# sephiroce/srf

Measured on AMD Instinct MI355X. Metric: acoustic frames/sec through SRF (123-d fbank, 3-iter DR) at 1/2/4/8 MI355X, higher is better.
Workload: dtype fp32; 1 GPU; wsj_c4: SRF L=6 PH=CH=16 DIM=32 LPAD=RPAD=2 DR iter=3, train step (fwd+bwd+allreduce+Adam); utterances_per_gpu=28, frames_per_utterance=800, global_batch=28, parallelism=dp1, launch=hipgraph (fwd+CTC+bwd)

## Files before the change

srf_amd/csrc/cnnfe.hip:

```cpp
#include <algorithm>
#include <type_traits>
#include <cmath>
#include <cstdlib>

#include "srf_common.h"
#include "srf_reduce.h"
#include "srf_rng.h"
#include "../../include/srf.h"

namespace {

constexpr int C = 64;
constexpr float kBnEps = 1e-3f;
constexpr float kBnMomentum = 0.99f;

struct Dims {
  int B, T, Fin;
  int T1, F1, T2, F2;
  int pt1, pf1, pt2, pf2;
};

inline int same_out(int n) { return (n + 1) / 2; }
inline int same_pad_before(int n) {
  const int out = same_out(n);
// ... 167 lines not shown
                                                           const float* __restrict__ gamma,
                                                           const float* __restrict__ beta,
                                                           float* __restrict__ mmean, float* __restrict__ mvar,
                                                           int training, float* __restrict__ stats,
                                                           const float* __restrict__ ymax, int nymax) {
  __shared__ float sh[3][16][C];
  __shared__ float ysh[16], ab[2][C];
  const int c = threadIdx.x & (C - 1), r = threadIdx.x >> 6;
  if (ymax != nullptr) {
    float m = 0.f;
    for (int k = threadIdx.x; k < nymax; k += 1024) m = fmaxf(m, ymax[k]);
#pragma unroll
    for (int o = 32; o >= 1; o >>= 1) m = fmaxf(m, __shfl_xor(m, o, 64));
    if (c == 0) ysh[r] = m;
  }
  float n = 0.f, mu = 0.f, m2 = 0.f;
  if (training)
#pragma unroll 8
    for (int k = r; k < nparts; k += 16)
      chan_merge(n, mu, m2, part[((size_t)k * 3 + 0) * C + c], part[((size_t)k * 3 + 1) * C + c],
                 part[((size_t)k * 3 + 2) * C + c]);
  sh[0][r][c] = n; sh[1][r][c] = mu; sh[2][r][c] = m2;
  __syncthreads();
  if (r == 0) {
    float mean, var;
    if (training) {
      for (int q = 1; q < 16; ++q) chan_merge(n, mu, m2, sh[0][q][c], sh[1][q][c], sh[2][q][c]);
      mean = mu;
      var = m2 / n;
      mmean[c] = mmean[c] * kBnMomentum + mean * (1.f - kBnMomentum);
      mvar[c] = mvar[c] * kBnMomentum + (n > 1.f ? var * n / (n - 1.f) : var) * (1.f - kBnMomentum);
    } else {
      mean = mmean[c];
      var = mvar[c];
    }
    const float rstd = 1.f / sqrtf(var + kBnEps);
    const float scale = gamma[c] * rstd;
    const float shift = beta[c] - mean * scale;
    stats[0 * C + c] = mean;
    stats[1 * C + c] = rstd;
    stats[2 * C + c] = scale;
    stats[3 * C + c] = shift;
    ab[0][c] = fabsf(scale);
    ab[1][c] = fabsf(shift);
  }
  if (ymax == nullptr) return;
  __syncthreads();
  if (threadIdx.x == 0) {
    float y = ysh[0], sa = 0.f, sb = 0.f;
    for (int q = 1; q < 16; ++q) y = fmaxf(y, ysh[q]);
    for (int q = 0; q < C; ++q) {
      sa = fmaxf(sa, ab[0][q]);
      sb = fmaxf(sb, ab[1][q]);
    }
    const int e = srf_split_exp(sa * y + sb);
    stats[4 * C + 0] = srf_exp2i(e);
    stats[4 * C + 1] = srf_exp2i(-e);
  }
}

typedef __bf16 cbf8 __attribute__((ext_vector_type(8)));
typedef float cf16 __attribute__((ext_vector_type(16)));

__device__ __forceinline__ cf16 mfma32bf(const cbf8& a, const cbf8& b, const cf16& c) {
  return __builtin_amdgcn_mfma_f32_32x32x16_bf16(a, b, c, 0, 0, 0);
}
typedef _Float16 ch8 __attribute__((ext_vector_type(8)));
__device__ __forceinline__ cf16 mfma32h(const ch8& a, const ch8& b, const cf16& c) {
  return __builtin_amdgcn_mfma_f32_32x32x16_f16(a, b, c, 0, 0, 0);
}

__device__ __forceinline__ void split8v(const float (&v)[8], cbf8& p1, cbf8& p2, cbf8& p3) {
#pragma unroll
  for (int k = 0; k < 8; ++k) {
    const __bf16 a1 = (__bf16)v[k];
    const float r = v[k] - (float)a1;
    const __bf16 a2 = (__bf16)r;
    p1[k] = a1;
    p2[k] = a2;
    p3[k] = (__bf16)(r - (float)a2);
  }
}

__device__ __forceinline__ void pack_w2_f16_body(int idx, const float* __restrict__ ka, const float* __restrict__ kb,
                                                 _Float16* __restrict__ wp2, float* __restrict__ wsc) {
  const int n = idx >> 6, cin = idx & 63;
  const float* k = n < C ? ka : kb;
  const int co = n % C;
  float v[9], m = 0.f;
#pragma unroll
  for (int tap = 0; tap < 9; ++tap) {
    v[tap] = k[((size_t)tap * C + cin) * C + co];
    m = fmaxf(m, fabsf(v[tap]));
  }
#pragma unroll
  for (int o = 32; o >= 1; o >>= 1) m = fmaxf(m, __shfl_xor(m, o, 64));
  const int e = srf_split_exp(m);
  const float sc = srf_exp2i(e);
  const size_t plane = (size_t)9 * 2 * C * C;
#pragma unroll
  for (int tap = 0; tap < 9; ++tap) {
    _Float16 h1, h2;
    srf_split2h(v[tap] * sc, h1, h2);
    const size_t o = ((size_t)tap * 2 * C + n) * C + cin;
    wp2[o] = h1;
    wp2[plane + o] = h2;
  }
  if (cin == 0) wsc[n] = srf_exp2i(-e);
}

constexpr int kC2BStride = 24;
constexpr int kC2Waves = 4;
constexpr int kC2Px = 32 * kC2Waves;
constexpr int kC2BLoads = 2 * 2 * C * 2 / (64 * kC2Waves);

__global__ __launch_bounds__(64 * kC2Waves) __attribute__((amdgpu_waves_per_eu(2))) void conv2_fwd32_kernel(
    const float* __restrict__ y1, const float* __restrict__ stats1, const int* __restrict__ inp_len, Dims d,
    const _Float16* __restrict__ wp2, const float* __restrict__ wsc, const float* __restrict__ ba,
    const float* __restrict__ bb, int training, float drop_p, unsigned long long seed,
    const unsigned long long* __restrict__ seed_src, float* __restrict__ y2, unsigned char* __restrict__ sel2,
    float* __restrict__ part) {
  seed = srf_step_seed(seed, seed_src);
  __shared__ __attribute__((aligned(16))) _Float16 Bs[2][2][2 * C * kC2BStride];
  __shared__ __attribute__((aligned(16))) float ss[2][C];
  __shared__ float red[3][kC2Waves][2 * 32];
  const int tid = threadIdx.x;
  const int lane = tid & 63, wv = tid >> 6;
  const int r = lane & 31, h = lane >> 5;
  const int P2 = d.B * d.T2 * d.F2;
  const int p0 = blockIdx.x * kC2Px;
  const size_t plane = (size_t)9 * 2 * C * C;
  if (tid < 2 * C) ss[tid >> 6][tid & 63] = stats1[(2 + (tid >> 6)) * C + (tid & 63)] * stats1[4 * C];

  const int pa = p0 + 32 * wv + r;
  const bool alive = pa < P2;
  const int pc = min(pa, P2 - 1);
  const int af2 = pc % d.F2, at2 = (pc / d.F2) % d.T2, ab = pc / (d.F2 * d.T2);
  const int alen1 = ceil_div_len(inp_len[ab], 2);

  auto load_b = [&](int kk, ch8 (&bv)[kC2BLoads]) {
    const int tap = kk >> 2, kb = kk & 3;
#pragma unroll
    for (int q = 0; q < kC2BLoads; ++q) {
      const int idx = q * 64 * kC2Waves + tid;
      const int pl = idx >> 8, rem = idx & 255, n = rem >> 1, half = rem & 1;
      bv[q] = *reinterpret_cast<const ch8*>(wp2 + pl * plane + ((size_t)tap * 2 * C + n) * C + 16 * kb + 8 * half);
    }
  };
  auto store_b = [&](int buf, const ch8 (&bv)[kC2BLoads]) {
#pragma unroll
    for (int q = 0; q < kC2BLoads; ++q) {
      const int idx = q * 64 * kC2Waves + tid;
      const int pl = idx >> 8, rem = idx & 255, n = rem >> 1, half = rem & 1;
      *reinterpret_cast<ch8*>(&Bs[buf][pl][n * kC2BStride + 8 * half]) = bv[q];
    }
  };
  auto load_a = [&](int kk, f4 (&av)[2], bool& ok) {
    const int tap = kk >> 2, kb = kk & 3;
    const int dt = tap / 3, df = tap - dt * 3;
    const int t1 = 2 * at2 - d.pt2 + dt, f1 = 2 * af2 - d.pf2 + df;
    ok = alive && t1 >= 0 && t1 < d.T1 && f1 >= 0 && f1 < d.F1 && t1 < alen1;
    const int t1c = min(max(t1, 0), d.T1 - 1), f1c = min(max(f1, 0), d.F1 - 1);
    const float* src = y1 + (((size_t)ab * d.T1 + t1c) * d.F1 + f1c) * C + 16 * kb + 8 * h;
    av[0] = *reinterpret_cast<const f4*>(src);
    av[1] = *reinterpret_cast<const f4*>(src + 4);
  };

  cf16 acc[4];
#pragma unroll
  for (int nt = 0; nt < 4; ++nt) acc[nt] = cf16{};
  auto compute = [&](int kk, int buf, const f4 (&av)[2], bool aok) {
    ch8 a1, a2;
    {
      const int c0 = 16 * (kk & 3) + 8 * h;
#pragma unroll
      for (int q = 0; q < 8; ++q) {
        const float x = q < 4 ? av[0][q] : av[1][q - 4];
        _Float16 h1, h2;
        srf_split2h(aok ? x * ss[0][c0 + q] + ss[1][c0 + q] : 0.f, h1, h2);
        a1[q] = h1;
        a2[q] = h2;
      }
    }
#pragma unroll
    for (int nt = 0; nt < 4; ++nt) {
      const int nrow = (nt >> 1) * C + 32 * (nt & 1) + r;
      const ch8 b1 = *reinterpret_cast<const ch8*>(&Bs[buf][0][nrow * kC2BStride + 8 * h]);
      const ch8 b2 = *reinterpret_cast<const ch8*>(&Bs[buf][1][nrow * kC2BStride + 8 * h]);
      cf16 c = acc[nt];
      c = mfma32h(a2, b1, c);
      c = mfma32h(a1, b2, c);
      c = mfma32h(a1, b1, c);
      acc[nt] = c;
    }
  };
  ch8 bvA[kC2BLoads], bvB[kC2BLoads];
  f4 avA[2], avB[2], avC[2];
  bool okA, okB, okC;
  load_b(0, bvA);
  load_a(0, avA, okA);
  load_b(1, bvB);
  load_a(1, avB, okB);
  store_b(0, bvA);
  __syncthreads();
  for (int kk = 0; kk < 36; kk += 2) {
    {
      const f4 a0[2] = {avA[0], avA[1]};
      const bool ok0 = okA;
      if (kk + 2 < 36) {
        load_b(kk + 2, bvA);
        load_a(kk + 2, avA, okA);
      }
      compute(kk, 0, a0, ok0);
      store_b(1, bvB);
      __syncthreads();
    }
    {
      const f4 a1v[2] = {avB[0], avB[1]};
      const bool ok1 = okB;
      if (kk + 3 < 36) {
        load_b(kk + 3, bvB);
        load_a(kk + 3, avB, okB);
      }
      compute(kk + 1, 1, a1v, ok1);
      if (kk + 2 < 36) store_b(0, bvA);
      __syncthreads();
    }
  }
  (void)avC;
  (void)okC;

  const float keep_scale = 1.f / (1.f - drop_p);
  const float inv_b = stats1[4 * C + 1];
#pragma unroll
  for (int g = 0; g < 2; ++g) {
    const int c = 32 * g + r;
    const float bia = ba[c], bib = bb[c];
    const float sca = wsc[c] * inv_b, scb = wsc[C + c] * inv_b;
    float n = 0.f, mean = 0.f, m2 = 0.f;
#pragma unroll
    for (int q = 0; q < 4; ++q)
#pragma unroll
      for (int v = 0; v < 4; ++v) {
        const int p = p0 + 32 * wv + 8 * q + 4 * h + v;
        if (p >= P2) continue;
        const int t2 = (p / d.F2) % d.T2, b = p / (d.F2 * d.T2);
        const size_t o = (size_t)p * C + c;
        float a = acc[g][4 * q + v] * sca + bia, bvv = acc[2 + g][4 * q + v] * scb + bib;
        if (training && drop_p > 0.f) {
          bool ka, kb;
          srf_keep2(seed, kStreamConv1a, o, drop_p, ka, kb);
          a *= ka ? keep_scale : 0.f;
          bvv *= kb ? keep_scale : 0.f;
        }
        const bool sel = a >= bvv;
        float y = sel ? a : bvv;
        if (t2 >= ceil_div_len(inp_len[b], 4)) y = 0.f;
        y2[o] = y;
        sel2[o] = sel ? 1 : 0;
        n += 1.f;
        const float delta = y - mean;
        mean += delta / n;
        m2 += delta * (y - mean);
      }
    {
      float nb, mb, qb, x;
      xpair32(n, x, nb);
      nb = h ? x : nb;
      xpair32(mean, x, mb);
      mb = h ? x : mb;
      xpair32(m2, x, qb);
      qb = h ? x : qb;
      if (h == 0) chan_merge(n, mean, m2, nb, mb, qb);
    }
    if (h == 0) {
      red[0][wv][g * 32 + r] = n;
      red[1][wv][g * 32 + r] = mean;
      red[2][wv][g * 32 + r] = m2;
    }
  }
  __syncthreads();
  if (tid < 2 * 32) {
    const int gc = tid;
    float n = red[0][0][gc], mean = red[1][0][gc], m2 = red[2][0][gc];
#pragma unroll
    for (int w = 1; w < kC2Waves; ++w) chan_merge(n, mean, m2, red[0][w][gc], red[1][w][gc], red[2][w][gc]);
    part[((size_t)blockIdx.x * 3 + 0) * C + gc] = n;
    part[((size_t)blockIdx.x * 3 + 1) * C + gc] = mean;
    part[((size_t)blockIdx.x * 3 + 2) * C + gc] = m2;
  }
}

__global__ void bn_apply_kernel(const float* __restrict__ y, const float* __restrict__ stats,
                                const int* __restrict__ inp_len, int B, int Tk, int Fk, int div,
                                float* __restrict__ out) {
  const int n4 = B * Tk * Fk * C / 4;
  for (int q = blockIdx.x * blockDim.x + threadIdx.x; q < n4; q += gridDim.x * blockDim.x) {
    const int c4 = (q * 4) % C;
    const int p = q * 4 / C;
    const int t = (p / Fk) % Tk;
    const int b = p / (Fk * Tk);
    f4 v = {0.f, 0.f, 0.f, 0.f};
    if (t < ceil_div_len(inp_len[b], div)) {
      const f4 x = reinterpret_cast<const f4*>(y)[q];
      v = x * *reinterpret_cast<const f4*>(stats + 2 * C + c4) + *reinterpret_cast<const f4*>(stats + 3 * C + c4);
    }
    reinterpret_cast<f4*>(out)[q] = v;
  }
}


constexpr int kBnPx = 16;
__device__ __forceinline__ f4 wave_sum_px(f4 v) {
#pragma unroll
  for (int o = 16; o <= 32; o <<= 1) {
    v.x += __shfl_xor(v.x, o, 64); v.y += __shfl_xor(v.y, o, 64);
    v.z += __shfl_xor(v.z, o, 64); v.w += __shfl_xor(v.w, o, 64);
  }
  return v;
}

__global__ __launch_bounds__(256) void bn_bwd_reduce_kernel(const float* __restrict__ g, const float* __restrict__ y,
                                                            const float* __restrict__ stats,
                                                            const int* __restrict__ inp_len, int B, int Tk, int Fk,
                                                            int div, float* __restrict__ part) {
  __shared__ f4 sh[2][4][C / 4];
  const int lane = threadIdx.x & 63, q = lane & 15, pg = lane >> 4;
  const int wave = __builtin_amdgcn_readfirstlane(threadIdx.x >> 6);
  const f4 mean = reinterpret_cast<const f4*>(stats)[q], rstd = reinterpret_cast<const f4*>(stats + C)[q];
  const int P = B * Tk * Fk;
  f4 s0 = {0.f, 0.f, 0.f, 0.f}, s1 = s0;
  for (int p0 = (blockIdx.x * 4 + wave) * kBnPx; p0 < P; p0 += gridDim.x * 4 * kBnPx) {
    constexpr int U = kBnPx / 4;
    f4 dy[U], yv[U];
    float m[U];
#pragma unroll
    for (int u = 0; u < U; ++u) {
      const int pu = p0 + 4 * u + pg;
      const int p = min(pu, P - 1);
      const int t = (p / Fk) % Tk;
// ... 35 lines not shown
    __bf16* __restrict__ wq3, _Float16* __restrict__ wq2h, float* __restrict__ wdsc, float* __restrict__ gmax) {
  if ((int)blockIdx.x >= nprep) {
    const int idx = (blockIdx.x - nprep) * blockDim.x + threadIdx.x;
    if (wq2h != nullptr) {
      if (idx < kPackW2tF16Threads) pack_w2t_f16_body(idx, pk_a, pk_b, wq2h, wdsc);
    } else if (idx < kPackW2tThreads) {
      pack_w2t_split_body(idx, pk_a, pk_b, wq3);
    }
    return;
  }
  seed = srf_step_seed(seed, seed_src);
  __shared__ f4 sh[2][4][C / 4];
  __shared__ float smax[4];
  const int lane = threadIdx.x & 63, q = lane & 15, pg = lane >> 4;
  const int wave = __builtin_amdgcn_readfirstlane(threadIdx.x >> 6);
  const int P = d.B * d.T2 * d.F2;
  const f4 mean = reinterpret_cast<const f4*>(stats2)[q], rstd = reinterpret_cast<const f4*>(stats2 + C)[q];
  const f4 gam = {gamma2[4 * q], gamma2[4 * q + 1], gamma2[4 * q + 2], gamma2[4 * q + 3]};
  const f4 sdy_n = reinterpret_cast<const f4*>(bnsum2)[q] / (float)P;
  const f4 sdyxh_n = reinterpret_cast<const f4*>(bnsum2 + C)[q] / (float)P;
  const float keep_scale = 1.f / (1.f - drop_p);
  f4 ga_s = {0.f, 0.f, 0.f, 0.f}, gb_s = ga_s;
  float gm = 0.f;
  for (int p0 = (blockIdx.x * 4 + wave) * kBnPx; p0 < P; p0 += nprep * 4 * kBnPx) {
    constexpr int U = kBnPx / 4;
    f4 gv[U], yv[U];
    unsigned sv[U];
    float m[U];
#pragma unroll
    for (int u = 0; u < U; ++u) {
      const int pu = p0 + 4 * u + pg;
      const int p = min(pu, P - 1);
      const int t = (p / d.F2) % d.T2;
      const int b = p / (d.F2 * d.T2);
      m[u] = (pu < P && t < ceil_div_len(inp_len[b], 4)) ? 1.f : 0.f;
      gv[u] = reinterpret_cast<const f4*>(g_out)[(size_t)p * (C / 4) + q];
      yv[u] = reinterpret_cast<const f4*>(y2)[(size_t)p * (C / 4) + q];
      sv[u] = reinterpret_cast<const unsigned*>(sel2)[(size_t)p * (C / 4) + q];
    }
#pragma unroll
    for (int u = 0; u < U; ++u) {
      const int pu = p0 + 4 * u + pg;
      if (pu >= P) continue;
      const size_t o0 = (size_t)pu * C + 4 * q;
      f4 ga, gb;
#pragma unroll
      for (int e = 0; e < 4; ++e) {
        const float gy = bn_bwd_elem(gv[u][e], yv[u][e], m[u], mean[e], rstd[e], gam[e], sdy_n[e], sdyxh_n[e]);
        const bool sel = ((sv[u] >> (8 * e)) & 0xffu) != 0;
        float a = sel ? gy : 0.f, bb = sel ? 0.f : gy;
        if (drop_p > 0.f) {
          bool ka, kb;
          srf_keep2(seed, kStreamConv1a, o0 + e, drop_p, ka, kb);
          a *= ka ? keep_scale : 0.f;
          bb *= kb ? keep_scale : 0.f;
        }
        ga[e] = a;
        gb[e] = bb;
        gm = fmaxf(gm, fmaxf(fabsf(a), fabsf(bb)));
      }
      reinterpret_cast<f4*>(g_ab + (size_t)pu * 2 * C)[q] = ga;
      reinterpret_cast<f4*>(g_ab + (size_t)pu * 2 * C + C)[q] = gb;
      ga_s += ga;
      gb_s += gb;
    }
  }
  ga_s = wave_sum_px(ga_s);
  gb_s = wave_sum_px(gb_s);
  if (pg == 0) { sh[0][wave][q] = ga_s; sh[1][wave][q] = gb_s; }
#pragma unroll
  for (int o = 32; o >= 1; o >>= 1) gm = fmaxf(gm, __shfl_xor(gm, o, 64));
  if (lane == 0) smax[wave] = gm;
  __syncthreads();
  if (threadIdx.x < 2 * (C / 4)) {
    const int k = threadIdx.x / (C / 4), qq = threadIdx.x % (C / 4);
    const f4 v = sh[k][0][qq] + sh[k][1][qq] + sh[k][2][qq] + sh[k][3][qq];
    reinterpret_cast<f4*>(part + (size_t)blockIdx.x * 2 * C + k * C)[qq] = v;
  }
  if (threadIdx.x == 0 && gmax != nullptr) gmax[blockIdx.x] = fmaxf(fmaxf(smax[0], smax[1]), fmaxf(smax[2], smax[3]));
}

struct DgCls {
  int boff[5];
};

__device__ __forceinline__ void pack_w2t_split_body(int idx, const float* __restrict__ ka,
                                                    const float* __restrict__ kb, __bf16* __restrict__ wq3) {
  const int n8 = idx % (2 * C / 8), cin = (idx / (2 * C / 8)) % C, tap = idx / (C * (2 * C / 8));
  const int n = 8 * n8;
  const float* k = (n < C ? ka : kb) + ((size_t)tap * C + cin) * C + (n % C);
  float v[8];
#pragma unroll
  for (int q = 0; q < 8; ++q) v[q] = k[q];
  cbf8 p1, p2, p3;
  split8v(v, p1, p2, p3);
  const size_t plane = (size_t)9 * C * 2 * C;
  const size_t o = ((size_t)tap * C + cin) * 2 * C + n;
  *reinterpret_cast<cbf8*>(wq3 + o) = p1;
  *reinterpret_cast<cbf8*>(wq3 + plane + o) = p2;
  *reinterpret_cast<cbf8*>(wq3 + 2 * plane + o) = p3;
}

__device__ __forceinline__ void pack_w2t_f16_body(int idx, const float* __restrict__ ka, const float* __restrict__ kb,
                                                  _Float16* __restrict__ wq2h, float* __restrict__ wdsc) {
  const int cin = idx >> 6, l = idx & 63;
  float v[9][2], m = 0.f;
#pragma unroll
  for (int tap = 0; tap < 9; ++tap)
#pragma unroll
    for (int u = 0; u < 2; ++u) {
      const int n = 2 * l + u;
      v[tap][u] = (n < C ? ka : kb)[((size_t)tap * C + cin) * C + (n % C)];
      m = fmaxf(m, fabsf(v[tap][u]));
    }
#pragma unroll
  for (int o = 32; o >= 1; o >>= 1) m = fmaxf(m, __shfl_xor(m, o, 64));
  const int e = srf_split_exp(m);
  const float sc = srf_exp2i(e);
  const size_t plane = (size_t)9 * C * 2 * C;
#pragma unroll
  for (int tap = 0; tap < 9; ++tap) {
    _Float16 h1[2], h2[2];
#pragma unroll
    for (int u = 0; u < 2; ++u) srf_split2h(v[tap][u] * sc, h1[u], h2[u]);
    const size_t o = ((size_t)tap * C + cin) * 2 * C + 2 * l;
    wq2h[o] = h1[0];
    wq2h[o + 1] = h1[1];
    wq2h[plane + o] = h2[0];
    wq2h[plane + o + 1] = h2[1];
  }
  if (l == 0) wdsc[cin] = srf_exp2i(-e);
}

constexpr int kD2Waves = 4;
constexpr int kD2Px = 32 * kD2Waves;

__device__ __forceinline__ int gab_exp(const float* __restrict__ gmax, int n) {
  __shared__ float wmx[16];
  const int tid = threadIdx.x, nw = (blockDim.x + 63) >> 6;
  float m = 0.f;
  for (int k = tid; k < n; k += blockDim.x) m = fmaxf(m, gmax[k]);
#pragma unroll
  for (int o = 32; o >= 1; o >>= 1) m = fmaxf(m, __shfl_xor(m, o, 64));
  if ((tid & 63) == 0) wmx[tid >> 6] = m;
  __syncthreads();
  for (int k = 0; k < nw; ++k) m = fmaxf(m, wmx[k]);
  return srf_split_exp(m);
}

template <bool H>
__global__ __launch_bounds__(64 * kD2Waves) __attribute__((amdgpu_waves_per_eu(2))) void conv2_dgrad32_kernel(
    const float* __restrict__ g_ab, const void* __restrict__ wqv, Dims d, DgCls cls, float* __restrict__ g_x1,
    const float* __restrict__ gmax, int ngmax, const float* __restrict__ wdsc) {
  using BT = std::conditional_t<H, _Float16, __bf16>;
  using V8 = std::conditional_t<H, ch8, cbf8>;
  constexpr int NPL = H ? 2 : 3;
  constexpr int BCH = NPL * C * 2;
  const BT* __restrict__ wq3 = static_cast<const BT*>(wqv);
  __shared__ __attribute__((aligned(16))) BT Bs[2][NPL][C * kC2BStride];
  const int tid = threadIdx.x;
  const int lane = tid & 63, wv = tid >> 6;
  const int r = lane & 31, h = lane >> 5;
  const int bid = blockIdx.x;
  const int c = (bid >= cls.boff[1]) + (bid >= cls.boff[2]) + (bid >= cls.boff[3]);
  const int qt = c >> 1, qf = c & 1;
  const int nkt = (d.T1 - qt + 1) / 2, nkf = (d.F1 - qf + 1) / 2;
  const int Pc = d.B * nkt * nkf;
  const int q0 = (bid - cls.boff[c]) * kD2Px;
  const int dt0 = (qt + d.pt2) & 1, df0 = (qf + d.pf2) & 1;
  const int ntf = (3 - df0 + 1) / 2, ntt = (3 - dt0 + 1) / 2;
  const int nkb = ntt * ntf * 8;
  const size_t plane = (size_t)9 * C * 2 * C;
  float sa = 1.f, inv_sa = 1.f;
  if constexpr (H) {
    const int ea = gab_exp(gmax, ngmax);
    sa = srf_exp2i(ea);
    inv_sa = srf_exp2i(-ea);
  }

  const int pa = q0 + 32 * wv + r;
  const bool alive = pa < Pc;
  const int pcl = min(pa, Pc - 1);
  const int akf = pcl % nkf, akt = (pcl / nkf) % nkt, ab = pcl / (nkf * nkt);
  const int at1 = qt + 2 * akt, af1 = qf + 2 * akf;
  auto tap_of = [&](int k) { return (dt0 + 2 * (k / ntf)) * 3 + df0 + 2 * (k % ntf); };

  constexpr int NBL = (BCH + 64 * kD2Waves - 1) / (64 * kD2Waves);
  auto load_b = [&](int kk, V8 (&bv)[NBL]) {
    const int tap = tap_of(kk >> 3), kb = kk & 7;
#pragma unroll
    for (int q = 0; q < NBL; ++q) {
      const int idx = min(q * 64 * kD2Waves + tid, BCH - 1);
      const int pl = idx / (2 * C), rem = idx % (2 * C), cin = rem >> 1, half = rem & 1;
      bv[q] = *reinterpret_cast<const V8*>(wq3 + pl * plane + ((size_t)tap * C + cin) * 2 * C + 16 * kb + 8 * half);
    }
  };
  auto store_b = [&](int buf, const V8 (&bv)[NBL]) {
#pragma unroll
    for (int q = 0; q < NBL; ++q) {
      const int idx = q * 64 * kD2Waves + tid;
      if (idx < BCH) {
        const int pl = idx / (2 * C), rem = idx % (2 * C), cin = rem >> 1, half = rem & 1;
        *reinterpret_cast<V8*>(&Bs[buf][pl][cin * kC2BStride + 8 * half]) = bv[q];
      }
    }
  };
  auto load_a = [&](int kk, f4 (&av)[2], bool& ok) {
    const int tap = tap_of(kk >> 3), kb = kk & 7;
    const int dt = tap / 3, df = tap - dt * 3;
    const int t2 = (at1 + d.pt2 - dt) >> 1, f2 = (af1 + d.pf2 - df) >> 1;
    ok = alive && t2 >= 0 && t2 < d.T2 && f2 >= 0 && f2 < d.F2;
    const int t2c = min(max(t2, 0), d.T2 - 1), f2c = min(max(f2, 0), d.F2 - 1);
    const float* src = g_ab + (((size_t)ab * d.T2 + t2c) * d.F2 + f2c) * 2 * C + 16 * kb + 8 * h;
    av[0] = *reinterpret_cast<const f4*>(src);
    av[1] = *reinterpret_cast<const f4*>(src + 4);
  };

  cf16 acc[2];
  acc[0] = cf16{};
  acc[1] = cf16{};
  auto compute = [&](int buf, const f4 (&av)[2], bool aok) {
    if constexpr (H) {
      ch8 a1, a2;
#pragma unroll
      for (int q = 0; q < 8; ++q) {
        const float v = aok ? (q < 4 ? av[0][q] : av[1][q - 4]) : 0.f;
        _Float16 h1, h2;
        srf_split2h(v * sa, h1, h2);
        a1[q] = h1;
        a2[q] = h2;
      }
#pragma unroll
      for (int nt = 0; nt < 2; ++nt) {
        const int nrow = 32 * nt + r;
        const ch8 b1 = *reinterpret_cast<const ch8*>(&Bs[buf][0][nrow * kC2BStride + 8 * h]);
        const ch8 b2 = *reinterpret_cast<const ch8*>(&Bs[buf][1][nrow * kC2BStride + 8 * h]);
        cf16 cc = acc[nt];
        cc = mfma32h(a2, b1, cc);
        cc = mfma32h(a1, b2, cc);
        cc = mfma32h(a1, b1, cc);
        acc[nt] = cc;
      }
      return;
    } else {
    cbf8 a1, a2, a3;
    {
      float v[8];
#pragma unroll
      for (int q = 0; q < 8; ++q) v[q] = aok ? (q < 4 ? av[0][q] : av[1][q - 4]) : 0.f;
      split8v(v, a1, a2, a3);
    }
#pragma unroll
    for (int nt = 0; nt < 2; ++nt) {
      const int nrow = 32 * nt + r;
      const cbf8 b1 = *reinterpret_cast<const cbf8*>(&Bs[buf][0][nrow * kC2BStride + 8 * h]);
      const cbf8 b2 = *reinterpret_cast<const cbf8*>(&Bs[buf][1][nrow * kC2BStride + 8 * h]);
      const cbf8 b3 = *reinterpret_cast<const cbf8*>(&Bs[buf][2][nrow * kC2BStride + 8 * h]);
      cf16 cc = acc[nt];
      cc = mfma32bf(a3, b1, cc);
      cc = mfma32bf(a1, b3, cc);
      cc = mfma32bf(a2, b2, cc);
      cc = mfma32bf(a2, b1, cc);
      cc = mfma32bf(a1, b2, cc);
      cc = mfma32bf(a1, b1, cc);
      acc[nt] = cc;
    }
    }
  };
  V8 bvA[NBL], bvB[NBL];
  f4 avA[2], avB[2];
  bool okA, okB;
  load_b(0, bvA);
  load_a(0, avA, okA);
  load_b(1, bvB);
  load_a(1, avB, okB);
  store_b(0, bvA);
  __syncthreads();
  for (int kk = 0; kk < nkb; kk += 2) {
    {
      const f4 a0[2] = {avA[0], avA[1]};
      const bool ok0 = okA;
      if (kk + 2 < nkb) {
        load_b(kk + 2, bvA);
        load_a(kk + 2, avA, okA);
      }
      compute(0, a0, ok0);
      store_b(1, bvB);
      __syncthreads();
    }
    {
      const f4 a1v[2] = {avB[0], avB[1]};
      const bool ok1 = okB;
      if (kk + 3 < nkb) {
        load_b(kk + 3, bvB);
        load_a(kk + 3, avB, okB);
      }
      compute(1, a1v, ok1);
      if (kk + 2 < nkb) store_b(0, bvA);
      __syncthreads();
    }
  }
  float osc[2] = {1.f, 1.f};
  if constexpr (H) {
    osc[0] = inv_sa * wdsc[r];
    osc[1] = inv_sa * wdsc[32 + r];
  }
#pragma unroll
  for (int q = 0; q < 4; ++q)
#pragma unroll
    for (int v = 0; v < 4; ++v) {
      const int p = q0 + 32 * wv + 8 * q + 4 * h + v;
      if (p >= Pc) continue;
      const int kf = p % nkf, kt = (p / nkf) % nkt, b = p / (nkf * nkt);
      float* dst = g_x1 + (((size_t)b * d.T1 + qt + 2 * kt) * d.F1 + qf + 2 * kf) * C + r;
      dst[0] = H ? acc[0][4 * q + v] * osc[0] : acc[0][4 * q + v];
      dst[32] = H ? acc[1][4 * q + v] * osc[1] : acc[1][4 * q + v];
    }
}

constexpr int kWgChunk = 32;

struct WgDiv {
  FastDiv f2, t2;
};

constexpr int kTpPx = 64;
template <bool H>
__global__ __launch_bounds__(256) void gab_split_t_kernel(const float* __restrict__ g_ab, int P2, int P2p,
                                                          void* __restrict__ gsTv, const float* __restrict__ gmax,
                                                          int ngmax) {
  __shared__ float tile[kTpPx][2 * C + 1];
  const int tid = threadIdx.x;
  const int p0 = blockIdx.x * kTpPx;
  float sa = 1.f;
  if constexpr (H) sa = srf_exp2i(gab_exp(gmax, ngmax));
  for (int k = tid; k < kTpPx * (2 * C / 4); k += 256) {
    const int px = k / (2 * C / 4), q = k % (2 * C / 4);
    const int p = p0 + px;
    const f4 v = p < P2 ? *reinterpret_cast<const f4*>(g_ab + (size_t)p * 2 * C + 4 * q) : f4{0.f, 0.f, 0.f, 0.f};
    tile[px][4 * q] = v.x;
    tile[px][4 * q + 1] = v.y;
    tile[px][4 * q + 2] = v.z;
    tile[px][4 * q + 3] = v.w;
  }
  __syncthreads();
  const size_t plane = (size_t)2 * C * P2p;
  for (int task = tid; task < 2 * C * (kTpPx / 8); task += 256) {
    const int o = task & 7, n = task >> 3;
    float v[8];
#pragma unroll
    for (int k = 0; k < 8; ++k) v[k] = tile[8 * o + k][n];
    if constexpr (H) {
      ch8 p1, p2;
#pragma unroll
      for (int k = 0; k < 8; ++k) {
        _Float16 h1, h2;
        srf_split2h(v[k] * sa, h1, h2);
        p1[k] = h1;
        p2[k] = h2;
      }
      _Float16* dst = static_cast<_Float16*>(gsTv) + (size_t)n * P2p + p0 + 8 * o;
      *reinterpret_cast<ch8*>(dst) = p1;
      *reinterpret_cast<ch8*>(dst + plane) = p2;
    } else {
      cbf8 p1, p2, p3;
      split8v(v, p1, p2, p3);
      __bf16* dst = static_cast<__bf16*>(gsTv) + (size_t)n * P2p + p0 + 8 * o;
      *reinterpret_cast<cbf8*>(dst) = p1;
      *reinterpret_cast<cbf8*>(dst + plane) = p2;
      *reinterpret_cast<cbf8*>(dst + 2 * plane) = p3;
    }
  }
}

constexpr int kW2Chunk = 32;
constexpr int kW2AStride = 96;

typedef short ws4 __attribute__((ext_vector_type(4)));

template <typename BT>
__device__ __forceinline__ ws4 lds_tr16(const BT* p) {
  return __builtin_amdgcn_ds_read_tr16_b64_v4i16(
      (__attribute__((address_space(3))) ws4*)(reinterpret_cast<uintptr_t>(p)));
}

template <bool H>
__global__ __launch_bounds__(256) __attribute__((amdgpu_waves_per_eu(2))) void conv2_wgrad32_kernel(
    const float* __restrict__ y1, const float* __restrict__ stats1, const int* __restrict__ inp_len,
    const void* __restrict__ gsTv, int P2p, Dims d, WgDiv dv, int nsplit, int split_len, float* __restrict__ part,
    const float* __restrict__ gmax, int ngmax) {
  using BT = std::conditional_t<H, _Float16, __bf16>;
  using V8 = std::conditional_t<H, ch8, cbf8>;
  constexpr int NPL = H ? 2 : 3;
  const BT* __restrict__ gsT3 = static_cast<const BT*>(gsTv);
  __shared__ __attribute__((aligned(16))) BT As[2][NPL][kW2Chunk * kW2AStride];
  float out_sc = 1.f;
// ... 460 lines not shown
  };
  const size_t op1 = take((size_t)conv1_blocks(d) * 3 * C * 4), op2 = take(nb2 * 3 * C * 4),
               owp = take((size_t)9 * 2 * C * C * 4), omg = take((size_t)kBnMerge * 3 * C * 4),
               owp2 = take((size_t)2 * 9 * 2 * C * C * 2), owsc = take((size_t)2 * C * 4),
               oym = take((size_t)conv1_blocks(d) * 4);
  char* b = static_cast<char*>(base);
  FwdWs w;
  w.wp2 = (_Float16*)(b + owp2);
  w.wsc = (float*)(b + owsc);
  w.ymax = (float*)(b + oym);
  w.merged = (float*)(b + omg);
  w.part1 = (float*)(b + op1);
  w.part2 = (float*)(b + op2);
  w.wp = (float*)(b + owp);
  w.bytes = off;
  return w;
}

int check_dims(int B, int T, int Fin, int nfilt) {
  SRF_REQUIRE(B > 0 && T > 0 && Fin > 0, "bad CNN-FE shape B=%d T=%d F=%d", B, T, Fin);
  SRF_REQUIRE(nfilt == C, "model-conv-filter-num must be %d (got %d)", C, nfilt);
  return SRF_OK;
}

}

extern "C" {

int srf_cnnfe_out_dims(int T, int feat_dim, int* T2, int* F2) {
  SRF_REQUIRE(T > 0 && feat_dim > 0 && T2 && F2, "bad arguments");
  Dims d = make_dims(1, T, feat_dim);
  *T2 = d.T2;
  *F2 = d.F2;
  return SRF_OK;
}

size_t srf_cnnfe_saved_bytes(int B, int T, int feat_dim, int nfilt) {
  (void)nfilt;
  return saved_layout(make_dims(B, T, feat_dim), nullptr).bytes;
}

size_t srf_cnnfe_fwd_workspace(int B, int T, int feat_dim, int nfilt) {
  (void)nfilt;
  return fwd_ws_layout(make_dims(B, T, feat_dim), nullptr).bytes;
}

int srf_cnnfe_fwd(const float* feats, const int* inp_len, int B, int T, int feat_dim, int nfilt,
                  const float* k0a, const float* b0a, const float* k0b, const float* b0b, const float* gamma0,
                  const float* beta0, const float* k1a, const float* b1a, const float* k1b, const float* b1b,
                  const float* gamma1, const float* beta1, float* mmean0, float* mvar0, float* mmean1, float* mvar1,
                  int training, float drop_p, unsigned long long seed, float* out, void* saved, size_t saved_bytes,
                  void* workspace, size_t workspace_bytes, void* stream) {
  int rc = check_dims(B, T, feat_dim, nfilt);
  if (rc) return rc;
  SRF_REQUIRE(feats && inp_len && k0a && b0a && k0b && b0b && gamma0 && beta0 && k1a && b1a && k1b && b1b &&
                  gamma1 && beta1 && mmean0 && mvar0 && mmean1 && mvar1 && out && saved && workspace,
              "null pointer argument");
  SRF_REQUIRE(drop_p >= 0.f && drop_p < 1.f, "dropout rate %f out of [0,1)", drop_p);
  const Dims d = make_dims(B, T, feat_dim);
  FwdSaved sv = saved_layout(d, saved);
  FwdWs w = fwd_ws_layout(d, workspace);
  if (saved_bytes < sv.bytes || workspace_bytes < w.bytes) {
    srf::set_error("CNN-FE buffers too small (saved %zu < %zu or workspace %zu < %zu)", saved_bytes, sv.bytes,
                   workspace_bytes, w.bytes);
    return SRF_EWORKSPACE;
  }
  hipStream_t st = static_cast<hipStream_t>(stream);
  const size_t P2 = (size_t)d.B * d.T2 * d.F2;
  const int nb2 = (int)((P2 + 63) / 64);
  int nparts2 = nb2;
  const int npack = (kPackW2Threads + 64 * kRows1 - 1) / (64 * kRows1);
  hipLaunchKernelGGL(conv1_fwd_kernel, dim3(conv1_blocks(d) + npack), dim3(64 * kRows1), conv1_lds(d), st, feats,
                     inp_len, d, k0a, b0a, k0b, b0b, training, drop_p, seed, srf::seed_source(), sv.y1, sv.sel1,
                     w.part1, conv1_blocks(d), k1a, k1b, w.wp2, w.wsc, w.ymax);
  SRF_LAUNCH_CHECK("conv1_fwd");
  if ((rc = bn_finalize(w.part1, conv1_blocks(d), w.merged, gamma0, beta0, mmean0, mvar0, training, sv.stats1, st,
                        w.ymax, conv1_blocks(d))))
    return rc;
  SRF_LAUNCH_CHECK("bn_finalize(1)");
  {
    const int nb32 = (int)((P2 + kC2Px - 1) / kC2Px);
    hipLaunchKernelGGL(conv2_fwd32_kernel, dim3(nb32), dim3(64 * kC2Waves), 0, st, sv.y1, sv.stats1, inp_len, d,
                       w.wp2, w.wsc, b1a, b1b, training, drop_p, seed, srf::seed_source(), sv.y2, sv.sel2,
                       w.part2);
    SRF_LAUNCH_CHECK("conv2_fwd32");
    nparts2 = nb32;
  }
  if ((rc = bn_finalize(w.part2, nparts2, w.merged, gamma1, beta1, mmean1, mvar1, training, sv.stats2, st)))
    return rc;
  SRF_LAUNCH_CHECK("bn_finalize(2)");
  hipLaunchKernelGGL(bn_apply_kernel, dim3(1024), dim3(256), 0, st, sv.y2, sv.stats2, inp_len, d.B, d.T2, d.F2, 4,
                     out);
  SRF_LAUNCH_CHECK("bn_apply");
  return SRF_OK;
}

}

namespace {
struct BwdWs2 {
  float *bnpart, *bnsum2, *bnsum1, *g_ab, *biaspart, *g_x1, *wq, *wpart, *c1part, *c1sum, *scratch;
  __bf16* gsT3;
  float* gmax;
  float* wdsc;
  int P2p;
  size_t bytes;
};

constexpr int kBnBlocks = 1024;
constexpr int kWgrad32SplitsMax = 128;
constexpr int kWgrad32Splits = 56;
inline bool wgrad_by_rows(const Dims& d) { return SRF_CONV2_WGRAD_ROWS && d.F2 <= 32; }

BwdWs2 bwd_ws_layout(const Dims& d, void* base) {
  const size_t P1 = (size_t)d.B * d.T1 * d.F1, P2 = (size_t)d.B * d.T2 * d.F2;
  size_t off = 0;
  auto take = [&](size_t bytes) {
    size_t o = off;
    off += srf::align_up(bytes, 256);
    return o;
  };
  const size_t obp = take((size_t)kBnBlocks * 2 * C * 4), os2 = take(2 * C * 4), os1 = take(2 * C * 4),
               oab = take(P2 * 2 * C * 4), obias = take((size_t)kBnBlocks * 2 * C * 4), ogx = take(P1 * C * 4),
               owq = take((size_t)9 * 2 * C * C * 4),
               owp = take((size_t)std::max(kWgrad32SplitsMax, kWrRanges) * 9 * C * 2 * C * 4),
               oc1 = take((size_t)conv1_blocks(d) * 20 * C * 4), oc1s = take(20 * C * 4),
               oscr = take(srf::colsum_scratch_floats(std::max(conv1_blocks(d), kBnBlocks), 20 * C) * 4);
  const int P2p = (int)((P2 + kTpPx - 1) / kTpPx * kTpPx);
  const size_t ogs3 = take(wgrad_by_rows(d) ? 0 : (size_t)3 * 2 * C * P2p * 2);
  const size_t ogm = take((size_t)kBnBlocks * 4), ods = take((size_t)C * 4);
  char* b = static_cast<char*>(base);
  BwdWs2 w;
  w.bnpart = (float*)(b + obp);
  w.bnsum2 = (float*)(b + os2);
  w.bnsum1 = (float*)(b + os1);
  w.g_ab = (float*)(b + oab);
  w.biaspart = (float*)(b + obias);
  w.g_x1 = (float*)(b + ogx);
  w.wq = (float*)(b + owq);
  w.wpart = (float*)(b + owp);
  w.c1part = (float*)(b + oc1);
  w.c1sum = (float*)(b + oc1s);
  w.scratch = (float*)(b + oscr);
  w.gsT3 = (__bf16*)(b + ogs3);
  w.gmax = (float*)(b + ogm);
  w.wdsc = (float*)(b + ods);
  w.P2p = P2p;
  w.bytes = off;
  return w;
}

}

extern "C" {

size_t srf_cnnfe_bwd_workspace(int B, int T, int feat_dim, int nfilt) {
  (void)nfilt;
  return bwd_ws_layout(make_dims(B, T, feat_dim), nullptr).bytes;
}

int srf_cnnfe_bwd(const float* feats, const int* inp_len, int B, int T, int feat_dim, int nfilt, const float* gamma0,
                  const float* k1a, const float* k1b, const float* gamma1, float drop_p, unsigned long long seed,
                  const void* saved, const float* g_out, float* g_k0a, float* g_b0a, float* g_k0b, float* g_b0b,
                  float* g_gamma0, float* g_beta0, float* g_k1a, float* g_b1a, float* g_k1b, float* g_b1b,
                  float* g_gamma1, float* g_beta1, void* workspace, size_t workspace_bytes, void* stream) {
  return srf_cnnfe_bwd_parts(SRF_CNNFE_BWD_ALL, feats, inp_len, B, T, feat_dim, nfilt, gamma0, k1a, k1b, gamma1, drop_p,
                             seed, saved, g_out, g_k0a, g_b0a, g_k0b, g_b0b, g_gamma0, g_beta0, g_k1a, g_b1a, g_k1b,
                             g_b1b, g_gamma1, g_beta1, workspace, workspace_bytes, stream);
}

int srf_cnnfe_bwd_parts(int parts, const float* feats, const int* inp_len, int B, int T, int feat_dim, int nfilt,
                        const float* gamma0, const float* k1a, const float* k1b, const float* gamma1, float drop_p,
                        unsigned long long seed, const void* saved, const float* g_out, float* g_k0a, float* g_b0a,
                        float* g_k0b, float* g_b0b, float* g_gamma0, float* g_beta0, float* g_k1a, float* g_b1a,
                        float* g_k1b, float* g_b1b, float* g_gamma1, float* g_beta1, void* workspace,
                        size_t workspace_bytes, void* stream) {
  SRF_REQUIRE(parts > 0 && (parts & ~SRF_CNNFE_BWD_ALL) == 0, "CNN-FE backward: bad parts mask %d", parts);
  int rc = check_dims(B, T, feat_dim, nfilt);
  if (rc) return rc;
  SRF_REQUIRE(feats && inp_len && gamma0 && k1a && k1b && gamma1 && saved && g_out && g_k0a && g_b0a && g_k0b &&
                  g_b0b && g_gamma0 && g_beta0 && g_k1a && g_b1a && g_k1b && g_b1b && g_gamma1 && g_beta1 &&
                  workspace,
              "null pointer argument");
  SRF_REQUIRE(((uintptr_t)g_out & 15) == 0 && ((uintptr_t)saved & 255) == 0 && ((uintptr_t)workspace & 255) == 0,
              "CNN-FE backward: g_out must be 16-byte and saved / workspace 256-byte aligned");
  const Dims d = make_dims(B, T, feat_dim);
  FwdSaved sv = saved_layout(d, const_cast<void*>(saved));
  BwdWs2 w = bwd_ws_layout(d, workspace);
  if (workspace_bytes < w.bytes) {
    srf::set_error("CNN-FE backward workspace too small: %zu < %zu", workspace_bytes, w.bytes);
    return SRF_EWORKSPACE;
  }
  hipStream_t st = static_cast<hipStream_t>(stream);
  const int P2 = d.B * d.T2 * d.F2;
  __bf16* wq3 = reinterpret_cast<__bf16*>(w.wq);
  _Float16* wq2h = reinterpret_cast<_Float16*>(w.wq);
  if (parts & SRF_CNNFE_BWD_PREP) {
  hipLaunchKernelGGL(bn_bwd_reduce_kernel, dim3(kBnBlocks), dim3(256), 0, st, g_out, sv.y2, sv.stats2, inp_len, d.B,
                     d.T2, d.F2, 4, w.bnpart);
  SRF_LAUNCH_CHECK("bn_bwd_reduce(2)");
  if ((rc = srf::colsum(w.bnpart, kBnBlocks, 2 * C, w.bnsum2, w.scratch, st, srf::ColSplit{{g_beta1, g_gamma1, nullptr, nullptr}, {C, C, 0, 0}})))
    return rc;
  const int npack = (kPackW2tF16Threads + 255) / 256;
  hipLaunchKernelGGL(conv2_bwd_prep_kernel, dim3(kBnBlocks + npack), dim3(256), 0, st, g_out, sv.y2, sv.sel2,
                     sv.stats2, gamma1, w.bnsum2, inp_len, d, drop_p, seed, srf::seed_source(), w.g_ab, w.biaspart,
                     kBnBlocks, k1a, k1b, wq3, wq2h, w.wdsc, w.gmax);
  SRF_LAUNCH_CHECK("conv2_bwd_prep");
  if ((rc = srf::colsum(w.biaspart, kBnBlocks, 2 * C, nullptr, w.scratch, st, srf::ColSplit{{g_b1a, g_b1b, nullptr, nullptr}, {C, C, 0, 0}})))
    return rc;
  }
  if (parts & SRF_CNNFE_BWD_DATA) {
    DgCls cls{};
    for (int c = 0; c < 4; ++c) {
      const int qt = c >> 1, qf = c & 1;
      const int Pc = d.B * ((d.T1 - qt + 1) / 2) * ((d.F1 - qf + 1) / 2);
      cls.boff[c + 1] = cls.boff[c] + (Pc + kD2Px - 1) / kD2Px;
    }
    hipLaunchKernelGGL(conv2_dgrad32_kernel<true>, dim3(cls.boff[4]), dim3(64 * kD2Waves), 0, st, w.g_ab,
                       (const void*)wq2h, d, cls, w.g_x1, (const float*)w.gmax, kBnBlocks, (const float*)w.wdsc);
    SRF_LAUNCH_CHECK("conv2_dgrad32");
  }
  const WgDiv dv{make_fastdiv(d.F2), make_fastdiv(d.T2)};
  const int nsplit = kWgrad32Splits;
  if ((parts & SRF_CNNFE_BWD_WGRAD) && wgrad_by_rows(d)) {
    const int rows_per = (d.B * d.T2 + kWrRanges - 1) / kWrRanges;
    hipLaunchKernelGGL(conv2_wgrad_rows_kernel, dim3(2 * kWrRanges), dim3(256), 0, st, sv.y1, sv.stats1, inp_len,
                       (const float*)w.g_ab, d, rows_per, w.wpart, (const float*)w.gmax, kBnBlocks);
    SRF_LAUNCH_CHECK("conv2_wgrad_rows");
    hipLaunchKernelGGL(conv2_wgrad_reduce_rows_kernel, dim3(9 * C * 2 * C / 128), dim3(256), 0, st, w.wpart, g_k1a,
                       g_k1b);
    SRF_LAUNCH_CHECK("conv2_wgrad_reduce_rows");
  } else if (parts & SRF_CNNFE_BWD_WGRAD) {
    static_assert(kW2Chunk == kWgChunk, "wgrad splits are whole chunks");
    const int split_len = ((P2 + nsplit - 1) / nsplit + kWgChunk - 1) / kWgChunk * kWgChunk;
    hipLaunchKernelGGL(gab_split_t_kernel<true>, dim3(w.P2p / kTpPx), dim3(256), 0, st, w.g_ab, P2, w.P2p,
                       (void*)w.gsT3, (const float*)w.gmax, kBnBlocks);
    SRF_LAUNCH_CHECK("gab_split_t");
    hipLaunchKernelGGL(conv2_wgrad32_kernel<true>, dim3(9 * nsplit), dim3(256), 0, st, sv.y1, sv.stats1, inp_len,
                       (const void*)w.gsT3, w.P2p, d, dv, nsplit, split_len, w.wpart, (const float*)w.gmax,
                       kBnBlocks);
    SRF_LAUNCH_CHECK("conv2_wgrad32");
    hipLaunchKernelGGL(conv2_wgrad_reduce_kernel, dim3((9 * C * 2 * C + 255) / 256), dim3(256), 0, st, w.wpart,
                       nsplit, g_k1a, g_k1b);
    SRF_LAUNCH_CHECK("conv2_wgrad_reduce");
  }
  if (!(parts & SRF_CNNFE_BWD_DATA)) return SRF_OK;
  hipLaunchKernelGGL(bn_bwd_reduce_kernel, dim3(kBnBlocks), dim3(256), 0, st, w.g_x1, sv.y1, sv.stats1, inp_len, d.B,
                     d.T1, d.F1, 2, w.bnpart);
  SRF_LAUNCH_CHECK("bn_bwd_reduce(1)");
  if ((rc = srf::colsum(w.bnpart, kBnBlocks, 2 * C, w.bnsum1, w.scratch, st, srf::ColSplit{{g_beta0, g_gamma0, nullptr, nullptr}, {C, C, 0, 0}})))
    return rc;
  hipLaunchKernelGGL(conv1_bwd_kernel, dim3(conv1_blocks(d)), dim3(64 * kRows1), conv1_lds(d), st, feats, inp_len, d, w.g_x1, sv.y1,
                     sv.sel1, sv.stats1, gamma0, w.bnsum1, drop_p, seed, srf::seed_source(), w.c1part);
  SRF_LAUNCH_CHECK("conv1_bwd");
  if ((rc = srf::colsum(w.c1part, conv1_blocks(d), 20 * C, nullptr, w.scratch, st,
                        srf::ColSplit{{g_k0a, g_k0b, g_b0a, g_b0b, nullptr, nullptr}, {9 * C, 9 * C, C, C, 0, 0}})))
    return rc;
  return SRF_OK;
}

}
```

Baseline: 3.098 million frames/s.

## Restructure conv2 fwd/dgrad k-loop pipeline with k-block-major weight packing

Repacks the conv2 forward and dgrad fp16 weight planes so each 16-channel k-block is contiguous. The main k-loops become a ring that prefetches activations NA blocks ahead and weights two blocks ahead. The forward input conversion now reads BN scale and shift as vector LDS loads, and the per-pixel divisions in the epilogues are replaced with precomputed fast divisions and a length mask. The aim is better latency hiding and fewer integer ops, at the cost of extra register pressure from the deeper A prefetch. The `min`-clamped prefetches redundantly reload the last block.

```diff
diff --git a/srf_amd/csrc/cnnfe.hip b/srf_amd/csrc/cnnfe.hip
--- a/srf_amd/csrc/cnnfe.hip
+++ b/srf_amd/csrc/cnnfe.hip
@@ -273,6 +273,16 @@
   }
 }
 
+#ifndef SRF_CONV2_PIPE
+#define SRF_CONV2_PIPE 1
+#endif
+#ifndef SRF_CONV2_FWD_NA
+#define SRF_CONV2_FWD_NA 2
+#endif
+#ifndef SRF_CONV2_DGRAD_NA
+#define SRF_CONV2_DGRAD_NA 2
+#endif
+
 __device__ __forceinline__ void pack_w2_f16_body(int idx, const float* __restrict__ ka, const float* __restrict__ kb,
                                                  _Float16* __restrict__ wp2, float* __restrict__ wsc) {
   const int n = idx >> 6, cin = idx & 63;
@@ -293,7 +303,11 @@
   for (int tap = 0; tap < 9; ++tap) {
     _Float16 h1, h2;
     srf_split2h(v[tap] * sc, h1, h2);
+#if SRF_CONV2_PIPE
+    const size_t o = (((size_t)tap * 4 + (cin >> 4)) * 2 * C + n) * 16 + (cin & 15);
+#else
     const size_t o = ((size_t)tap * 2 * C + n) * C + cin;
+#endif
     wp2[o] = h1;
     wp2[plane + o] = h2;
   }
@@ -304,13 +318,18 @@
 constexpr int kC2Waves = 4;
 constexpr int kC2Px = 32 * kC2Waves;
 constexpr int kC2BLoads = 2 * 2 * C * 2 / (64 * kC2Waves);
+struct C2Div {
+  FastDiv f2, ft;
+};
+constexpr int kC2ADepth = SRF_CONV2_FWD_NA;
+constexpr int kD2ADepth = SRF_CONV2_DGRAD_NA;
 
 __global__ __launch_bounds__(64 * kC2Waves) __attribute__((amdgpu_waves_per_eu(2))) void conv2_fwd32_kernel(
     const float* __restrict__ y1, const float* __restrict__ stats1, const int* __restrict__ inp_len, Dims d,
     const _Float16* __restrict__ wp2, const float* __restrict__ wsc, const float* __restrict__ ba,
     const float* __restrict__ bb, int training, float drop_p, unsigned long long seed,
     const unsigned long long* __restrict__ seed_src, float* __restrict__ y2, unsigned char* __restrict__ sel2,
-    float* __restrict__ part) {
+    float* __restrict__ part, C2Div dv) {
   seed = srf_step_seed(seed, seed_src);
   __shared__ __attribute__((aligned(16))) _Float16 Bs[2][2][2 * C * kC2BStride];
   __shared__ __attribute__((aligned(16))) float ss[2][C];
@@ -335,7 +354,13 @@
     for (int q = 0; q < kC2BLoads; ++q) {
       const int idx = q * 64 * kC2Waves + tid;
       const int pl = idx >> 8, rem = idx & 255, n = rem >> 1, half = rem & 1;
+#if SRF_CONV2_PIPE
+      bv[q] = *reinterpret_cast<const ch8*>(wp2 + pl * plane + ((size_t)kk * 2 * C + n) * 16 + 8 * half);
+      (void)tap;
+      (void)kb;
+#else
       bv[q] = *reinterpret_cast<const ch8*>(wp2 + pl * plane + ((size_t)tap * 2 * C + n) * C + 16 * kb + 8 * half);
+#endif
     }
   };
   auto store_b = [&](int buf, const ch8 (&bv)[kC2BLoads]) {
@@ -360,6 +385,7 @@
   cf16 acc[4];
 #pragma unroll
   for (int nt = 0; nt < 4; ++nt) acc[nt] = cf16{};
+#if !SRF_CONV2_PIPE
   auto compute = [&](int kk, int buf, const f4 (&av)[2], bool aok) {
     ch8 a1, a2;
     {
@@ -385,6 +411,62 @@
       acc[nt] = c;
     }
   };
+#else
+  auto convert = [&](int kk, const f4 (&av)[2], bool aok, ch8& a1, ch8& a2) {
+    const int c0 = 16 * (kk & 3) + 8 * h;
+    const f4 sc[2] = {*reinterpret_cast<const f4*>(&ss[0][c0]), *reinterpret_cast<const f4*>(&ss[0][c0 + 4])};
+    const f4 sh[2] = {*reinterpret_cast<const f4*>(&ss[1][c0]), *reinterpret_cast<const f4*>(&ss[1][c0 + 4])};
+#pragma unroll
+    for (int q = 0; q < 8; ++q) {
+      const float v = av[q >> 2][q & 3] * sc[q >> 2][q & 3] + sh[q >> 2][q & 3];
+      _Float16 h1, h2;
+      srf_split2h(aok ? v : 0.f, h1, h2);
+      a1[q] = h1;
+      a2[q] = h2;
+    }
+  };
+  auto mma = [&](int buf, const ch8& a1, const ch8& a2) {
+#pragma unroll
+    for (int nt = 0; nt < 4; ++nt) {
+      const int nrow = (nt >> 1) * C + 32 * (nt & 1) + r;
+      const ch8 b1 = *reinterpret_cast<const ch8*>(&Bs[buf][0][nrow * kC2BStride + 8 * h]);
+      const ch8 b2 = *reinterpret_cast<const ch8*>(&Bs[buf][1][nrow * kC2BStride + 8 * h]);
+      cf16 c = acc[nt];
+      c = mfma32h(a2, b1, c);
+      c = mfma32h(a1, b2, c);
+      c = mfma32h(a1, b1, c);
+      acc[nt] = c;
+    }
+  };
+  constexpr int NA = kC2ADepth;
+  static_assert(NA >= 2 && NA % 2 == 0 && 36 % NA == 0, "whole pairs; the ring repeats every NA k-blocks");
+  ch8 bv[2][kC2BLoads];
+  f4 av[NA][2];
+  bool ok[NA];
+  load_b(0, bv[0]);
+  load_b(1, bv[1]);
+#pragma unroll
+  for (int u = 0; u < NA; ++u) load_a(u, av[u], ok[u]);
+  store_b(0, bv[0]);
+  __syncthreads();
+  for (int kk = 0; kk < 36; kk += NA) {
+#pragma unroll
+    for (int u = 0; u < NA; ++u) {
+      const int k = kk + u;
+      ch8 a1, a2;
+      load_b(min(k + 2, 35), bv[u & 1]);
+      convert(k, av[u], ok[u], a1, a2);
+      if (u & 1) {
+        load_a(min(k - 1 + NA, 35), av[u - 1], ok[u - 1]);
+        load_a(min(k + NA, 35), av[u], ok[u]);
+      }
+      mma(u & 1, a1, a2);
+      store_b((u + 1) & 1, bv[(u + 1) & 1]);
+      __syncthreads();
+    }
+  }
+#endif
+#if !SRF_CONV2_PIPE
   ch8 bvA[kC2BLoads], bvB[kC2BLoads];
   f4 avA[2], avB[2], avC[2];
   bool okA, okB, okC;
@@ -420,9 +502,19 @@
   }
   (void)avC;
   (void)okC;
+#endif
 
   const float keep_scale = 1.f / (1.f - drop_p);
   const float inv_b = stats1[4 * C + 1];
+#if SRF_CONV2_PIPE
+  unsigned past = 0;
+#pragma unroll
+  for (int i = 0; i < 16; ++i) {
+    const int p = min(p0 + 32 * wv + 8 * (i >> 2) + 4 * h + (i & 3), P2 - 1);
+    const int b = (int)fdiv((unsigned)p, dv.ft), t2 = (int)fdiv((unsigned)p, dv.f2) - b * d.T2;
+    if (t2 >= ceil_div_len(inp_len[b], 4)) past |= 1u << i;
+  }
+#endif
 #pragma unroll
   for (int g = 0; g < 2; ++g) {
     const int c = 32 * g + r;
@@ -435,7 +527,9 @@
       for (int v = 0; v < 4; ++v) {
         const int p = p0 + 32 * wv + 8 * q + 4 * h + v;
         if (p >= P2) continue;
+#if !SRF_CONV2_PIPE
         const int t2 = (p / d.F2) % d.T2, b = p / (d.F2 * d.T2);
+#endif
         const size_t o = (size_t)p * C + c;
         float a = acc[g][4 * q + v] * sca + bia, bvv = acc[2 + g][4 * q + v] * scb + bib;
         if (training && drop_p > 0.f) {
@@ -446,7 +540,11 @@
         }
         const bool sel = a >= bvv;
         float y = sel ? a : bvv;
+#if SRF_CONV2_PIPE
+        if ((past >> (4 * q + v)) & 1) y = 0.f;
+#else
         if (t2 >= ceil_div_len(inp_len[b], 4)) y = 0.f;
+#endif
         y2[o] = y;
         sel2[o] = sel ? 1 : 0;
         n += 1.f;
@@ -648,6 +746,7 @@
 
 struct DgCls {
   int boff[5];
+  FastDiv fkf[2], fpx[4];
 };
 
 __device__ __forceinline__ void pack_w2t_split_body(int idx, const float* __restrict__ ka,
@@ -689,7 +788,11 @@
     _Float16 h1[2], h2[2];
 #pragma unroll
     for (int u = 0; u < 2; ++u) srf_split2h(v[tap][u] * sc, h1[u], h2[u]);
+#if SRF_CONV2_PIPE
+    const size_t o = (((size_t)tap * 8 + (l >> 3)) * C + cin) * 16 + (2 * l & 15);
+#else
     const size_t o = ((size_t)tap * C + cin) * 2 * C + 2 * l;
+#endif
     wq2h[o] = h1[0];
     wq2h[o + 1] = h1[1];
     wq2h[plane + o] = h2[0];
@@ -758,7 +861,12 @@
     for (int q = 0; q < NBL; ++q) {
       const int idx = min(q * 64 * kD2Waves + tid, BCH - 1);
       const int pl = idx / (2 * C), rem = idx % (2 * C), cin = rem >> 1, half = rem & 1;
+#if SRF_CONV2_PIPE
+      static_assert(H, "the bf16 planes keep [tap][cin][n]");
+      bv[q] = *reinterpret_cast<const V8*>(wq3 + pl * plane + (((size_t)tap * 8 + kb) * C + cin) * 16 + 8 * half);
+#else
       bv[q] = *reinterpret_cast<const V8*>(wq3 + pl * plane + ((size_t)tap * C + cin) * 2 * C + 16 * kb + 8 * half);
+#endif
     }
   };
   auto store_b = [&](int buf, const V8 (&bv)[NBL]) {
@@ -833,6 +941,35 @@
     }
     }
   };
+#if SRF_CONV2_PIPE
+  constexpr int NA = kD2ADepth;
+  static_assert(NA >= 2 && NA % 2 == 0 && 8 % NA == 0, "whole pairs; the ring repeats every NA k-blocks");
+  V8 bv[2][NBL];
+  f4 av[NA][2];
+  bool ok[NA];
+  load_b(0, bv[0]);
+  load_b(1, bv[1]);
+#pragma unroll
+  for (int u = 0; u < NA; ++u) load_a(u, av[u], ok[u]);
+  store_b(0, bv[0]);
+  __syncthreads();
+  for (int kk = 0; kk < nkb; kk += NA) {
+#pragma unroll
+    for (int u = 0; u < NA; ++u) {
+      const int k = kk + u;
+      const f4 a[2] = {av[u][0], av[u][1]};
+      const bool aok = ok[u];
+      load_b(min(k + 2, nkb - 1), bv[u & 1]);
+      compute(u & 1, a, aok);
+      if (u & 1) {
+        load_a(min(k - 1 + NA, nkb - 1), av[u - 1], ok[u - 1]);
+        load_a(min(k + NA, nkb - 1), av[u], ok[u]);
+      }
+      store_b((u + 1) & 1, bv[(u + 1) & 1]);
+      __syncthreads();
+    }
+  }
+#else
   V8 bvA[NBL], bvB[NBL];
   f4 avA[2], avB[2];
   bool okA, okB;
@@ -866,6 +1003,7 @@
       __syncthreads();
     }
   }
+#endif
   float osc[2] = {1.f, 1.f};
   if constexpr (H) {
     osc[0] = inv_sa * wdsc[r];
@@ -877,7 +1015,12 @@
     for (int v = 0; v < 4; ++v) {
       const int p = q0 + 32 * wv + 8 * q + 4 * h + v;
       if (p >= Pc) continue;
+#if SRF_CONV2_PIPE
+      const int b = (int)fdiv((unsigned)p, cls.fpx[c]), row = (int)fdiv((unsigned)p, cls.fkf[qf]);
+      const int kf = p - row * nkf, kt = row - b * nkt;
+#else
       const int kf = p % nkf, kt = (p / nkf) % nkt, b = p / (nkf * nkt);
+#endif
       float* dst = g_x1 + (((size_t)b * d.T1 + qt + 2 * kt) * d.F1 + qf + 2 * kf) * C + r;
       dst[0] = H ? acc[0][4 * q + v] * osc[0] : acc[0][4 * q + v];
       dst[32] = H ? acc[1][4 * q + v] * osc[1] : acc[1][4 * q + v];
@@ -1504,7 +1647,7 @@
     const int nb32 = (int)((P2 + kC2Px - 1) / kC2Px);
     hipLaunchKernelGGL(conv2_fwd32_kernel, dim3(nb32), dim3(64 * kC2Waves), 0, st, sv.y1, sv.stats1, inp_len, d,
                        w.wp2, w.wsc, b1a, b1b, training, drop_p, seed, srf::seed_source(), sv.y2, sv.sel2,
-                       w.part2);
+                       w.part2, C2Div{make_fastdiv(d.F2), make_fastdiv(d.T2 * d.F2)});
     SRF_LAUNCH_CHECK("conv2_fwd32");
     nparts2 = nb32;
   }
@@ -1637,6 +1780,8 @@
       const int qt = c >> 1, qf = c & 1;
       const int Pc = d.B * ((d.T1 - qt + 1) / 2) * ((d.F1 - qf + 1) / 2);
       cls.boff[c + 1] = cls.boff[c] + (Pc + kD2Px - 1) / kD2Px;
+      cls.fkf[qf] = make_fastdiv((d.F1 - qf + 1) / 2);
+      cls.fpx[c] = make_fastdiv(((d.T1 - qt + 1) / 2) * ((d.F1 - qf + 1) / 2));
     }
     hipLaunchKernelGGL(conv2_dgrad32_kernel<true>, dim3(cls.boff[4]), dim3(64 * kD2Waves), 0, st, w.g_ab,
                        (const void*)wq2h, d, cls, w.g_x1, (const float*)w.gmax, kBnBlocks, (const float*)w.wdsc);
```

New measurement: 3.126 million frames/s, median of 6. About the same (+0.9%).
